# CHEBSB/PolarDecoding

Measured on AMD Instinct MI355X. Metric: decoded frames/sec, N=1024 K=512 CA-SCL L=8, higher is better.
Workload: dtype f64

## Files before the change

include/polar_hip.h:

```cpp
#ifndef POLAR_HIP_H
#define POLAR_HIP_H

#include <stddef.h>
#include <stdint.h>

#ifdef __cplusplus
extern "C" {
#endif

#define POLAR_ALGO_SC 0
#define POLAR_ALGO_BP 1
#define POLAR_ALGO_SCL 2
#define POLAR_ALGO_CASCL 3
#define POLAR_ALGO_SCF 4
#define POLAR_ALGO_SCAN 5
#define POLAR_ALGO_BPL 6

#define POLAR_F64 0
#define POLAR_F32 1
#define POLAR_Q8 2

#define POLAR_OK 0
#define POLAR_EINVAL (-1)
#define POLAR_ENOMEM (-2)
// ... 102 lines not shown

int polar_bpl_set_graphs(polar_ctx *ctx, const int *perms, int P);
int polar_bpl_get_graphs(const polar_ctx *ctx, int *P, int *perms);
int polar_bpl_cyclic_graphs(int n, int P, int *out);
int polar_bpl_decode_device(polar_ctx *ctx, const void *d_in, int in_is_f32, double sigma, size_t B, uint32_t *d_uhat_bits,
                            uint32_t *d_iters, uint32_t *d_flags, uint32_t *d_graph, uint32_t *d_total_iters);
int polar_bpl_decode_batch(polar_ctx *ctx, const double *llr_in, size_t B, int *u_hat, unsigned *iters, unsigned *flags,
                           unsigned *graph, unsigned *total_iters);

#define POLAR_RM_NONE 0
#define POLAR_RM_REPEAT 1
#define POLAR_RM_PUNCTURE 2
#define POLAR_RM_SHORTEN 3
#define POLAR_RM_SHORT_LLR 1048576.0
int polar_rm_select_n(int A, int E, int n_max);
int polar_rm_info_order(int N, int A, int E, int *out);
int polar_create_rm(const polar_cfg *cfg, int E, int ibil, polar_ctx **out);
int polar_rm_info(const polar_ctx *ctx, int *E, int *mode, int *ibil);
int polar_rm_recover_device(polar_ctx *ctx, const void *d_in, int in_is_f32, double sigma, size_t B, void *d_out);

int polar_genie_count_device(polar_ctx *ctx, const void *d_in, int in_is_f32, double sigma, size_t B, uint64_t *d_counts);
int polar_genie_rows_device(polar_ctx *ctx, unsigned long long seed, unsigned long long first_frame, double sigma, size_t B,
                            void *d_out, int out_is_f32);
int polar_construct_batch(polar_ctx *ctx, unsigned long long seed, unsigned long long first_frame, double sigma, size_t B,
                          uint64_t *d_counts);
int polar_construct_order(int N, const uint64_t *counts, const int *base_order, int *out);

typedef struct polar_dyn {
    int D;
    const int *pos;
    const int *ptr;
    const int *idx;
} polar_dyn;
int polar_create_dyn(const polar_cfg *cfg, const polar_dyn *dyn, polar_ctx **out);
int polar_dyn_info(const polar_ctx *ctx, int *D, int *pos);
int polar_dyn_pac(int N, const int *info_order, int A, const int *g_taps, int n_taps, int *pos, int *ptr, int *idx,
                  int idx_cap, int *nnz);
int polar_pac_precode(int N, const int *g_taps, int n_taps, const int *v, size_t B, int *u);
int polar_pac_unprecode(int N, const int *g_taps, int n_taps, const int *u, size_t B, int *v);
int polar_dyn_pc5g(int N, const int *q_i, int n_qi, int n_pc, int n_pc_wm, int *pos, int *ptr, int *idx, int idx_cap,
                   int *nnz, int *info_order);


int polar_transform_device(polar_ctx *ctx, const uint32_t *d_in, size_t B, uint32_t *d_out);
int polar_encode_device(polar_ctx *ctx, const uint32_t *d_payload, size_t B, uint32_t *d_u_bits, uint32_t *d_x_bits);
int polar_payload_device(polar_ctx *ctx, const uint32_t *d_uhat_bits, size_t B, uint32_t *d_payload, uint32_t *d_crc_ok);
int polar_encode_batch(polar_ctx *ctx, const int *payload, size_t B, int *u, int *x);
int polar_payload_batch(polar_ctx *ctx, const int *u_hat, size_t B, int *payload, unsigned *crc_ok);
int polar_set_systematic(polar_ctx *ctx, int on);
int polar_get_systematic(const polar_ctx *ctx);
int polar_systematic_check(int N, const int *info_order, int A);
int polar_crc_masks(int N, const int *info_order, int A, int crc_r, const int *crc_taps, int n_taps, int systematic,
                    uint32_t *crc_tab, uint32_t *masks);

int polar_q8_set_quant(polar_ctx *ctx, double scale, int qc, int qi);
int polar_q8_get_quant(const polar_ctx *ctx, double *scale, int *qc, int *qi);
int polar_q8_quantize_host(const double *in, size_t n, double sigma, double scale, int qc, int8_t *out);
int polar_q8_quantize_device(polar_ctx *ctx, const void *d_in, int in_is_f32, double sigma, size_t B, int8_t *d_out);
int polar_q8_decode_device(polar_ctx *ctx, const int8_t *d_q, size_t B, uint32_t *d_uhat_bits, int32_t *d_pm, uint32_t *d_flags);
int polar_q8_decode_batch(polar_ctx *ctx, const int8_t *q, size_t B, int *u_hat, int32_t *pm, unsigned *flags);

int polar_generate_device(polar_ctx *ctx, unsigned long long seed, unsigned long long first_frame, double snr_db,
                          size_t B, void *d_out, int out_is_f32, int out_is_y, uint32_t *d_u_bits);

int polar_fer_batch(polar_ctx *ctx, unsigned long long seed, unsigned long long first_frame, double snr_db, size_t B,
                    unsigned long long *block_errors, unsigned long long *bit_errors);

typedef struct polar_group polar_group;
int polar_group_create(const polar_cfg *cfg, int ngpus, polar_group **out);
void polar_group_destroy(polar_group *grp);
int polar_group_size(const polar_group *grp);
int polar_group_fer_batch(polar_group *grp, unsigned long long seed, unsigned long long first_frame, double snr_db,
                          size_t frames_per_gpu, unsigned long long *block_errors, unsigned long long *bit_errors,
                          double *seconds);
int polar_group_stop_rule_batch(polar_group *grp, unsigned long long seed, unsigned long long first_frame, double snr_db,
                                size_t frames_per_gpu, unsigned need, size_t min_frames, size_t *frames_used,
                                unsigned long long *block_errors, unsigned long long *bit_errors);
int polar_fer_multi_gpu(const polar_cfg *cfg, int ngpus, unsigned long long seed, unsigned long long first_frame,
                        double snr_db, size_t frames_per_gpu, unsigned long long *block_errors,
                        unsigned long long *bit_errors, double *seconds);

int polar_set_stream(polar_ctx *ctx, void *hip_stream);
void *polar_get_stream(polar_ctx *ctx);
int polar_synchronize(polar_ctx *ctx);

int polar_time_decode_device(polar_ctx *ctx, const void *d_in, int in_is_f32, double sigma, size_t B,
                             uint32_t *d_uhat_bits, int reps, float *ms_per_launch);

int polar_info_order(const polar_ctx *ctx, int *out, int n);
int polar_ctx_info(const polar_ctx *ctx, int *N, int *K, int *A, int *L, int *algo, int *dtype);
const char *polar_kernel_name(const polar_ctx *ctx);
const char *polar_version(void);

#ifdef __cplusplus
}
#endif
#endif
```

polardecoding_amd/csrc/polar_hip.hip:

```cpp
#include "polar_host.h"
#ifdef POLAR_TESTING
#include "../../include/polar_hip_testing.h"
#endif

#include <dlfcn.h>

#include <chrono>
#include <cmath>
#include <cstdio>
#include <cstdlib>
#include <mutex>
#include <thread>

#include "count_kernel.h"
#include "gen_kernel.h"
#include "scf_params.h"
#include "scan_params.h"

namespace {

const int kQ5G[1024] = {
#include "q5g_table.inc"
};

std::vector<int> default_order(int N)
{
    std::vector<int> q;
    if (N <= 1024) {
        for (int i = 0; i < 1024; ++i)
            if (kQ5G[i] < N) q.push_back(kQ5G[i]);
    } else {
        int n = 0;
        while ((1 << n) < N) ++n;
        std::vector<std::pair<double, int>> w(N);
        const double beta = std::pow(2.0, 0.25);
        for (int i = 0; i < N; ++i) {
            double s = 0;
            for (int b = 0; b < n; ++b)
                if ((i >> b) & 1) s += std::pow(beta, b);
            w[i] = {s, i};
        }
        std::stable_sort(w.begin(), w.end());
        for (auto &x : w) q.push_back(x.second);
    }
    return q;
}

std::vector<uint32_t> make_crc_table(int N, int r, const std::vector<int> &taps, const std::vector<int> &I)
{
    std::vector<uint32_t> tab(N, 0u);
    uint64_t glow = 0;
    for (int t : taps)
        if (t < r) glow |= 1ull << t;
    const uint64_t top = 1ull << r;
    uint64_t rem = 1;
    if (r == 0) return tab;
    for (size_t i = 0; i < I.size(); ++i) {
        tab[I[i]] = (uint32_t)rem;
        rem <<= 1;
        if (rem & top) rem = (rem ^ top) ^ glow;
    }
    return tab;
}

std::vector<uint32_t> make_crc_masks(int N, const std::vector<uint32_t> &tab)
{
    std::vector<uint32_t> t = tab;
    for (int s = 1; s < N; s <<= 1)
        for (int k = 0; k < N; ++k)
            if (k & s) t[(size_t)k] ^= t[(size_t)(k ^ s)];
    const int NW = N / 32;
    std::vector<uint32_t> m((size_t)polar::CRC_MASK_ROWS * NW, 0u);
    for (int k = 0; k < N; ++k)
        for (int i = 0; i < polar::CRC_MASK_ROWS; ++i)
            if ((t[(size_t)k] >> i) & 1u) m[(size_t)i * NW + (k >> 5)] |= 1u << (k & 31);
    return m;
}

int upload_crc_tables(polar_ctx *c, const std::vector<uint32_t> &t)
{
    const std::vector<uint32_t> m = make_crc_masks(c->cfg.N, t);
    if (int rc = c->d_crc_tab.upload(t.data(), t.size())) return rc;
    return c->d_crc_mask.upload(m.data(), m.size());
}

size_t chunk_rows(const polar_ctx *c, size_t B, size_t row_bytes, size_t floor = 64)
{
    return std::min(B, std::max(floor, c->chunk_bytes / row_bytes));
}

bool has_crc(int algo) { return algo == POLAR_ALGO_CASCL || algo == POLAR_ALGO_SCF || algo == POLAR_ALGO_BPL; }

const int kRmP[32] = {0, 1, 2, 4, 3, 5, 6, 7, 8, 16, 9, 17, 10, 18, 11, 19, 12, 20, 13, 21, 14, 22, 15, 23, 24, 25, 26, 28, 27, 29, 30, 31};

int rm_J(int N, int n) { return kRmP[n / (N / 32)] * (N / 32) + n % (N / 32); }

bool rm_args_ok(int N, int A, int E)
{
    return N >= 32 && N <= 1024 && !(N & (N - 1)) && A >= 1 && E >= A && E <= 8192;
}

int rm_mode_of(int N, int A, int E)
{
    if (E >= N) return POLAR_RM_REPEAT;
    return (16 * A <= 7 * E) ? POLAR_RM_PUNCTURE : POLAR_RM_SHORTEN;
}

int rm_order(int N, int A, int E, std::vector<int> &I)
{
    if (!rm_args_ok(N, A, E)) return POLAR_EINVAL;
    std::vector<unsigned char> pre((size_t)N, 0);
    const int mode = rm_mode_of(N, A, E);
    if (mode == POLAR_RM_PUNCTURE) {
        for (int n = 0; n < N - E; ++n) pre[(size_t)rm_J(N, n)] = 1;
        const int t = (4 * E >= 3 * N) ? (3 * N - 2 * E + 3) / 4 : (9 * N - 4 * E + 15) / 16;
        for (int i = 0; i < t; ++i) pre[(size_t)i] = 1;
    } else if (mode == POLAR_RM_SHORTEN) {
        for (int n = E; n < N; ++n) pre[(size_t)rm_J(N, n)] = 1;
    }
    const std::vector<int> q = default_order(N);
    I.clear();
    for (int i = N - 1; i >= 0 && (int)I.size() < A; --i)
        if (!pre[(size_t)q[(size_t)i]]) I.push_back(q[(size_t)i]);
    if ((int)I.size() < A) return POLAR_EINVAL;
    std::reverse(I.begin(), I.end());
    return POLAR_OK;
}

std::vector<uint16_t> rm_channel_ilv(int E)
// ... 103 lines not shown

int q8_decode_rows(polar_ctx *c, const void *d_in, int in_is_f32, double sigma, size_t B, uint32_t *d_bits, double *d_pm,
                   uint32_t *d_flags)
{
    const size_t esz = in_is_f32 ? 4 : 8;
    if (reinterpret_cast<uintptr_t>(d_in) % esz) return POLAR_EINVAL;
    const size_t N = (size_t)c->cfg.N;
    const size_t CH = chunk_rows(c, B, N);
    int rc;
    if ((rc = ensure(c, c->q8_rows, CH * N))) return rc;
    if (d_pm && (rc = ensure(c, c->q8_pm, CH * sizeof(int32_t)))) return rc;
    for (size_t off = 0; off < B; off += CH) {
        const size_t nc = std::min(CH, B - off);
        int8_t *rows = (int8_t *)c->q8_rows.p;
        int32_t *pm = d_pm ? (int32_t *)c->q8_pm.p : nullptr;
        if ((rc = polar_tu::q8_quantize(c, (const char *)d_in + off * N * esz, in_is_f32 != 0, sigma, nc * N, rows))) return rc;
        if ((rc = polar_tu::q8_decode(c, rows, nc, d_bits + off * (size_t)c->NW, pm, d_flags ? d_flags + off : nullptr))) return rc;
        if (d_pm && (rc = polar_tu::q8_pm_f64(c, pm, nc, d_pm + off))) return rc;
    }
    return POLAR_OK;
}

int decode_fixed(polar_ctx *c, const void *d_in, int in_is_f32, double sigma, size_t B, uint32_t *d_bits,
                 double *d_pm, uint32_t *d_flags, const uint32_t *d_frozen, uint32_t *d_iters = nullptr)
{
    if (!c || !d_in || !d_bits) return POLAR_EINVAL;
    if (B == 0) return POLAR_OK;
    if (B > 0x7fffffffull) return POLAR_EINVAL;
    const polar_cfg &g = c->cfg;
    if (g.dtype == POLAR_Q8) return q8_decode_rows(c, d_in, in_is_f32, sigma, B, d_bits, d_pm, d_flags);
    const bool f32 = g.dtype == POLAR_F32;
    const Family fam = kernel_family(c, in_is_f32, B);
    if (fam == Family::BP) {
        polar::BpParams P{};
        P.in = d_in; P.sigma = sigma; P.out_bits = d_bits; P.frozen = d_frozen;
        P.N = g.N; P.n = c->n; P.B = (int)B; P.iters = g.bp_iters;
        if (d_pm) HIP_TRY(c, hipMemsetAsync(d_pm, 0, B * sizeof(double), c->stream));
        P.stop = c->bp_stop;
        if (P.stop != POLAR_BP_STOP_NONE) {
            P.iters_out = d_iters;
            P.flags_out = d_flags;
        } else {
            if (d_flags) HIP_TRY(c, hipMemsetAsync(d_flags, 0, B * sizeof(uint32_t), c->stream));
            if (d_iters) HIP_TRY(c, hipMemsetD32Async(reinterpret_cast<hipDeviceptr_t>(d_iters), g.bp_iters, B, c->stream));
        }
        return polar_tu::bp(c, P, f32, in_is_f32 != 0);
    }
    polar::SclParams P{};
    P.in = d_in; P.sigma = sigma; P.out_bits = d_bits; P.pm = d_pm; P.flags = d_flags;
    P.frozen = d_frozen;
    P.crc_tab = (g.algo == POLAR_ALGO_CASCL) ? c->d_crc_tab : nullptr;
    P.crc_mask = (g.algo == POLAR_ALGO_CASCL) ? c->d_crc_mask : nullptr;
    P.crc_r = (g.algo == POLAR_ALGO_CASCL) ? g.crc_r : 0;
    P.N = g.N; P.n = c->n; P.B = (int)B;
    P.sc_mode = (g.algo == POLAR_ALGO_SC) ? 1 : 0;
    P.dbg = nullptr;
    P.scratch = nullptr;
    P.queue = nullptr;
    const bool in32 = in_is_f32 != 0;
    const bool crc = g.algo == POLAR_ALGO_CASCL;
    switch (fam) {
    case Family::WIDE: return polar_tu::scl_wide(c, P, f32, in32);
    case Family::DYN: return polar_tu::scl_dyn(c, P, f32, in32);
    case Family::SC_LANES: return polar_tu::sc_lanes(c, P, f32, in32);
#ifdef POLAR_TESTING
    case Family::FAST4: return polar_tu::scl_fast4(c, P, f32, in32, crc);
#endif
    case Family::FAST2: return polar_tu::scl_fast2(c, P, f32, in32, crc);
    case Family::FAST: return polar_tu::scl_fast(c, P, f32, in32, crc);
    case Family::BIG: return f32 ? polar_tu::scl_big_f32(c, P, in32) : polar_tu::scl_big_f64(c, P, in32);
    default: return polar_tu::scl_generic(c, P, f32, in32);
    }
}

void refresh_kernel_name(polar_ctx *c);
void sync_stage_ctx(polar_ctx *c)
{
    for (polar_ctx *s : c->stage_ctx) {
        if (!s) continue;
        s->stream.adopt(c->stream);
        s->force_generic = c->force_generic;
        s->force_spill = c->force_spill;
        s->use_fast2 = c->use_fast2;
        s->use_fast4 = c->use_fast4;
        s->big_split = c->big_split;
        s->chunk_bytes = c->chunk_bytes;
    }
}

int cascl_adaptive(polar_ctx *c, const void *d_in, int in_is_f32, double sigma, size_t B, uint32_t *d_bits,
                   double *d_pm, uint32_t *d_flags, uint32_t *d_list)
{
    hipStreamCaptureStatus cs = hipStreamCaptureStatusNone;
    HIP_TRY(c, hipStreamIsCapturing(c->stream, &cs));
    if (cs != hipStreamCaptureStatusNone) return POLAR_EINVAL;
    sync_stage_ctx(c);
    const std::vector<int> &st = c->cascl_stages;
    const int m = (int)st.size(), N = c->cfg.N, NW = c->NW;
    const size_t row = (size_t)N * (in_is_f32 ? 4 : 8);
    const size_t CH = chunk_rows(c, B, row);
    int rc;
    if (!d_flags) {
        if ((rc = ensure(c, c->ad_flags, B * sizeof(uint32_t)))) return rc;
        d_flags = (uint32_t *)c->ad_flags.p;
    }
    for (Buf *b : {&c->ad_idx[0], &c->ad_idx[1], &c->ad_sflags})
// ... 365 lines not shown
        }
        a += "; glue k_ad_crc_check, k_ad_fail_count/scan/write, k_ad_gather, k_ad_scatter";
        c->kernel_name = a;
    }
    if (c->rm_mode != POLAR_RM_NONE) c->kernel_name = "k_rm_recover, then " + c->kernel_name;
    if (fam == Family::DYN || (fam == Family::WIDE && c->is_dyn)) c->kernel_name = nm;
}

std::vector<uint32_t> pack_mask(const unsigned char *m, int N, bool invert)
{
    std::vector<uint32_t> w(N / 32, 0u);
    for (int j = 0; j < N; ++j)
        if ((m[j] != 0) != invert) w[j >> 5] |= 1u << (j & 31);
    return w;
}

void unpack_words(const uint32_t *w, int NW, int *out)
{
    struct Row { int v[8]; };
    static const std::vector<Row> tab = [] {
        std::vector<Row> t(256);
        for (int b = 0; b < 256; ++b)
            for (int k = 0; k < 8; ++k) t[(size_t)b].v[k] = (b >> k) & 1;
        return t;
    }();
    for (int i = 0; i < NW; ++i) {
        const uint32_t x = w[i];
        std::memcpy(out + 32 * i, &tab[x & 255u], sizeof(Row));
        std::memcpy(out + 32 * i + 8, &tab[(x >> 8) & 255u], sizeof(Row));
        std::memcpy(out + 32 * i + 16, &tab[(x >> 16) & 255u], sizeof(Row));
        std::memcpy(out + 32 * i + 24, &tab[x >> 24], sizeof(Row));
    }
}

constexpr unsigned HOST_THREADS = 6;
int host_batch(polar_ctx *c, const double *in, double sigma, const unsigned char *frozen_mask, size_t B,
               int *u_hat, double *pm_out, unsigned *flags, unsigned *iters = nullptr, unsigned *graph = nullptr,
               unsigned *total = nullptr, int *sets = nullptr)
{
    if (!c || !in || !u_hat) return POLAR_EINVAL;
    DeviceGuard guard(c->cfg.device);
    if (B == 0) return POLAR_OK;
    const int N = c->cfg.N, NW = c->NW;
    const int W = c->rm_mode != POLAR_RM_NONE ? c->rm_E : N;
    const uint32_t *d_frozen = c->d_frozen;
    if (frozen_mask) {
        if (has_crc(c->cfg.algo) || c->rm_mode != POLAR_RM_NONE || c->is_dyn || c->cfg.dtype == POLAR_Q8) return POLAR_EINVAL;
        std::vector<uint32_t> w = pack_mask(frozen_mask, N, false);
        if (!c->d_frozen_override) HIP_TRY(c, c->d_frozen_override.alloc((size_t)NW));
        HIP_TRY(c, hipMemcpyAsync(c->d_frozen_override, w.data(), NW * sizeof(uint32_t), hipMemcpyHostToDevice,
                                  c->stream));
        HIP_TRY(c, hipStreamSynchronize(c->stream));
        d_frozen = c->d_frozen_override;
    }
    int rc;
    if ((rc = ensure(c, c->pm, B * sizeof(double)))) return rc;
    if ((rc = ensure(c, c->flags, B * sizeof(uint32_t)))) return rc;
    if (iters && (rc = ensure(c, c->bp_iters, B * sizeof(uint32_t)))) return rc;
    if (graph && (rc = ensure(c, c->bpl_graph, B * sizeof(uint32_t)))) return rc;
    if (total && (rc = ensure(c, c->bpl_total, B * sizeof(uint32_t)))) return rc;
    if (sets && (rc = ensure(c, c->scf_hsets, B * polar::SCF_MAX_ORDER * sizeof(int32_t)))) return rc;
    const size_t CH = std::max<size_t>(256, std::min<size_t>(16384, ((size_t)128 << 20) / ((size_t)W * sizeof(double))));
    std::vector<size_t> off{0};
    {
        std::vector<size_t> head, tail;
        size_t left = B;
        if (B >= 6 * CH && CH >= 2048) {
            for (size_t d = 8; d >= 2; d /= 2) {
                head.push_back(CH / d);
                tail.insert(tail.begin(), CH / d);
                left -= 2 * (CH / d);
            }
        }
        for (size_t h : head) off.push_back(off.back() + h);
        while (left > 0) {
            const size_t nfc = std::min(CH, left);
            off.push_back(off.back() + nfc);
            left -= nfc;
        }
        for (size_t t : tail) off.push_back(off.back() + t);
    }
    const size_t nch = off.size() - 1;
    const size_t chf = std::min(B, CH);
    for (int i = 0; i < 2; ++i) {
        if ((rc = ensure(c, c->in2[i], chf * W * sizeof(double)))) return rc;
        if ((rc = ensure(c, c->bits2[i], chf * NW * sizeof(uint32_t)))) return rc;
    }
    const bool staged = nch >= 3;
    for (int i = 0; i < 2; ++i) {
        HIP_TRY(c, c->h_bits[i].ensure(chf * NW * sizeof(uint32_t)));
        if (staged) HIP_TRY(c, c->h_in[i].ensure(chf * W * sizeof(double)));
    }
    if (!c->copy_stream) {
        HIP_TRY(c, c->copy_stream.create(hipStreamNonBlocking));
        for (int i = 0; i < 2; ++i) {
            HIP_TRY(c, c->ev_in[i].create(hipEventDisableTiming));
            HIP_TRY(c, c->ev_free[i].create(hipEventDisableTiming));
            HIP_TRY(c, c->ev_out[i].create(hipEventDisableTiming));
        }
    }
    auto stage_chunk = [&](size_t k) {
        const size_t f0 = off[k], nf = off[k + 1] - off[k];
        const double *src = in + f0 * (size_t)W;
        double *dst = c->h_in[k & 1];
        const unsigned nthr = HOST_THREADS;
        auto part = [=](unsigned t) {
// ... 151 lines not shown
        std::vector<int> q = default_order(N);
        c->info_order.assign(q.end() - c->A, q.end());
    }
    c->cfg.info_order = c->info_order.data();
    c->frozen.assign(N, 1);
    for (int i = 0; i < c->A; ++i) {
        const int j = c->info_order[i];
        if (j < 0 || j >= N || c->frozen[j] == 0) { delete c; return POLAR_EINVAL; }
        c->frozen[j] = 0;
    }
    c->h_crc_tab = make_crc_table(N, r, c->taps, c->info_order);
    c->scf_T = std::min(8, c->A);

    int ndev = 0;
    if (hipGetDeviceCount(&ndev) != hipSuccess || cfg->device < 0 || cfg->device >= ndev) {
        delete c;
        return POLAR_EDEVICE;
    }
    DeviceGuard guard(cfg->device);
    hipDeviceProp_t prop;
    hipError_t e = hipGetDeviceProperties(&prop, cfg->device);
    if (e != hipSuccess) {
        delete c;
        return POLAR_EDEVICE;
    }
    c->num_cu = prop.multiProcessorCount;
    auto cleanup = [&](int rc) {
        polar_destroy(c);
        return rc;
    };
    if (c->stream.create(hipStreamNonBlocking) != hipSuccess) return cleanup(POLAR_EDEVICE);
    if (c->ev0.create(hipEventDefault) != hipSuccess || c->ev1.create(hipEventDefault) != hipSuccess) return cleanup(POLAR_EDEVICE);
    std::vector<uint32_t> fw = pack_mask(c->frozen.data(), N, false);
    std::vector<uint32_t> iw = pack_mask(c->frozen.data(), N, true);
    c->cfg.crc_systematic = (cfg->crc_systematic && r > 0) ? 1 : 0;
    if (c->cfg.crc_systematic) {
        std::fill(iw.begin(), iw.end(), 0u);
        for (int i = r; i < c->A; ++i) iw[c->info_order[i] >> 5] |= 1u << (c->info_order[i] & 31);
        std::vector<uint32_t> rows((size_t)cfg->K);
        uint64_t glow = 0;
        for (int t : c->taps)
            if (t < r) glow |= 1ull << t;
        const uint64_t top = 1ull << r;
        uint64_t rem = glow;
        for (int k = 0; k < cfg->K; ++k) {
            rows[(size_t)k] = (uint32_t)rem;
            rem <<= 1;
            if (rem & top) rem = (rem ^ top) ^ glow;
        }
        if (int rc = c->d_gc_rows.upload(rows.data(), rows.size())) return cleanup(rc);
    }
    if (c->d_frozen.alloc((size_t)c->NW) != hipSuccess || c->d_info.alloc((size_t)c->NW) != hipSuccess) return cleanup(POLAR_ENOMEM);
    if (int rc = c->d_frozen.upload(fw.data(), (size_t)c->NW)) return cleanup(rc);
    if (int rc = c->d_info.upload(iw.data(), (size_t)c->NW)) return cleanup(rc);
    if (r > 0)
        if (int rc = upload_crc_tables(c, c->h_crc_tab)) return cleanup(rc);
    if (cfg->algo == POLAR_ALGO_BPL) {
        c->bp_stop = POLAR_BP_STOP_G;
        const int P = std::min(c->n, 8);
        std::vector<int> perms((size_t)P * c->n);
        polar_bpl_cyclic_graphs(c->n, P, perms.data());
        if (int rc = polar_bpl_set_graphs(c, perms.data(), P)) return cleanup(rc);
    }
    refresh_kernel_name(c);
    *out = c;
    return POLAR_OK;
}

void polar_destroy(polar_ctx *c)
{
    if (!c) return;
    DeviceGuard guard(c->cfg.device);
    for (hipStream_t st : {c->stream.get(), c->copy_stream.get(), c->lane_b.stream.get()})
        if (st) (void)hipStreamSynchronize(st);
    for (polar_ctx *s : c->stage_ctx) polar_destroy(s);
    delete c;
}

int polar_set_stream(polar_ctx *c, void *s)
{
    if (!c) return POLAR_EINVAL;
    DeviceGuard guard(c->cfg.device);
    if (c->stream.is_owned()) (void)hipStreamSynchronize(c->stream);
    c->stream.adopt((hipStream_t)s);
    return POLAR_OK;
}

void *polar_get_stream(polar_ctx *c) { return c ? (void *)c->stream.get() : nullptr; }

int polar_synchronize(polar_ctx *c)
{
    if (!c) return POLAR_EINVAL;
    DeviceGuard guard(c->cfg.device);
    HIP_TRY(c, hipStreamSynchronize(c->stream));
    return POLAR_OK;
}

int polar_ctx_info(const polar_ctx *c, int *N, int *K, int *A, int *L, int *algo, int *dtype)
{
    if (!c) return POLAR_EINVAL;
    if (N) *N = c->cfg.N;
    if (K) *K = c->cfg.K;
    if (A) *A = c->A;
    if (L) *L = c->cfg.L;
    if (algo) *algo = c->cfg.algo;
    if (dtype) *dtype = c->cfg.dtype;
// ... 962 lines not shown
            if (j & s) t[(size_t)j] ^= t[(size_t)(j ^ s)];
    for (int j = 0; j < N; ++j)
        if (c->frozen[(size_t)j]) t[(size_t)j] = 0u;
}

}

int polar_systematic_check(int N, const int *info_order, int A)
{
    if (N < 32 || N > 4096 || (N & (N - 1)) || !info_order || A < 1 || A > N) return POLAR_EINVAL;
    const int NW = N / 32;
    std::vector<uint32_t> keep((size_t)NW, 0u);
    for (int i = 0; i < A; ++i) {
        const int j = info_order[i];
        if (j < 0 || j >= N || ((keep[(size_t)(j >> 5)] >> (j & 31)) & 1u)) return POLAR_EINVAL;
        keep[(size_t)(j >> 5)] |= 1u << (j & 31);
    }
    std::vector<uint32_t> w((size_t)NW);
    for (int i = 0; i < A; ++i) {
        const int j = info_order[i];
        std::fill(w.begin(), w.end(), 0u);
        w[(size_t)(j >> 5)] = 1u << (j & 31);
        host_transform(w.data(), NW);
        for (int k = 0; k < NW; ++k) w[(size_t)k] &= keep[(size_t)k];
        host_transform(w.data(), NW);
        for (int k = 0; k < NW; ++k)
            if ((w[(size_t)k] & keep[(size_t)k]) != (k == (j >> 5) ? 1u << (j & 31) : 0u)) return 0;
    }
    return 1;
}

int polar_crc_masks(int N, const int *info_order, int A, int crc_r, const int *crc_taps, int n_taps, int systematic,
                    uint32_t *crc_tab, uint32_t *masks)
{
    if (N < 32 || N > 4096 || (N & (N - 1)) || !info_order || A < 1 || A > N || crc_r < 1 || crc_r > 32 || !crc_taps ||
        n_taps < 2 || !masks)
        return POLAR_EINVAL;
    polar_ctx c;
    c.cfg.N = N;
    c.frozen.assign((size_t)N, 1);
    for (int i = 0; i < A; ++i) {
        if (info_order[i] < 0 || info_order[i] >= N) return POLAR_EINVAL;
        c.frozen[(size_t)info_order[i]] = 0;
    }
    c.h_crc_tab = make_crc_table(N, crc_r, std::vector<int>(crc_taps, crc_taps + n_taps), std::vector<int>(info_order, info_order + A));
    std::vector<uint32_t> t = c.h_crc_tab;
    if (systematic) make_crc_table_sys(&c, t);
    if (crc_tab) std::copy(t.begin(), t.end(), crc_tab);
    const std::vector<uint32_t> m = make_crc_masks(N, t);
    std::copy(m.begin(), m.end(), masks);
    return POLAR_OK;
}

int polar_get_systematic(const polar_ctx *c) { return c && c->sys_polar ? 1 : 0; }

int polar_set_systematic(polar_ctx *c, int on)
{
    if (!c || (on != 0 && on != 1)) return POLAR_EINVAL;
    if ((on != 0) == c->sys_polar) return POLAR_OK;
    if (on) {
        if (c->is_dyn || c->rm_mode != POLAR_RM_NONE || c->cfg.dtype == POLAR_Q8 || c->cfg.algo == POLAR_ALGO_BPL) return POLAR_EINVAL;
        if (polar_systematic_check(c->cfg.N, c->info_order.data(), c->A) != 1) return POLAR_EINVAL;
    }
    DeviceGuard guard(c->cfg.device);
    if (c->d_crc_tab) {
        if (c->h_crc_tab_sys.empty()) make_crc_table_sys(c, c->h_crc_tab_sys);
        const std::vector<uint32_t> &t = on ? c->h_crc_tab_sys : c->h_crc_tab;
        HIP_TRY(c, hipStreamSynchronize(c->stream));
        if (int rc = upload_crc_tables(c, t)) return rc;
        for (polar_ctx *s : c->stage_ctx)
            if (s && s->d_crc_tab)
                if (int rc = upload_crc_tables(s, t)) return rc;
    }
    c->sys_polar = on != 0;
    return POLAR_OK;
}

int polar_transform_device(polar_ctx *c, const uint32_t *d_in, size_t B, uint32_t *d_out)
{
    if (!c || !d_in || !d_out || B > 0x7fffffffull) return POLAR_EINVAL;
    DeviceGuard guard(c->cfg.device);
    return polar_tu::enc_transform(c, d_in, nullptr, false, B, d_out);
}

int polar_encode_device(polar_ctx *c, const uint32_t *d_payload, size_t B, uint32_t *d_u_bits, uint32_t *d_x_bits)
{
    if (!c || !d_payload || (!d_u_bits && !d_x_bits) || B > 0x7fffffffull) return POLAR_EINVAL;
    if (B == 0) return POLAR_OK;
    DeviceGuard guard(c->cfg.device);
    int rc;
    if ((rc = enc_tables(c))) return rc;
    const size_t row = (size_t)c->NW * sizeof(uint32_t);
    uint32_t *u = d_u_bits;
    if (!u) {
        if ((rc = ensure_nomem(c, c->enc_u, B * row, kEncScratch))) return rc;
        u = (uint32_t *)c->enc_u.p;
    }
    const bool rm = c->rm_mode != POLAR_RM_NONE;
    if (rm && d_x_bits && (rc = ensure_nomem(c, c->enc_x, B * row, kEncScratch))) return rc;
    if ((rc = polar_tu::enc_place(c, d_payload, B, u))) return rc;
    if (c->is_dyn && (rc = polar_tu::enc_dyn_fill(c, u, B))) return rc;
    if (c->sys_polar && (rc = polar_tu::enc_transform(c, u, nullptr, true, B, u))) return rc;
    if (!d_x_bits) return POLAR_OK;
    if (!rm) return polar_tu::enc_transform(c, u, nullptr, false, B, d_x_bits);
    if ((rc = polar_tu::enc_transform(c, u, nullptr, false, B, (uint32_t *)c->enc_x.p))) return rc;
    return polar_tu::enc_rm_select(c, (const uint32_t *)c->enc_x.p, B, d_x_bits);
// ... 432 lines not shown
```

polardecoding_amd/csrc/polar_host.h:

```cpp
#pragma once
#include "../../include/polar_hip.h"

#include <hip/hip_runtime.h>

#include <algorithm>
#include <cstdint>
#include <cstring>
#include <string>
#include <vector>

#include "dev_owned.h"
#include "polar_params.h"

namespace polar {
struct ScfParams;
struct GenParams;
struct ScanParams;
}

struct Lane {
    Stream stream;
    Buf scratch;
    Buf rm_rows;
    Buf q8_rows;
};

constexpr size_t kChunkBytes = (size_t)256 << 20;

struct polar_ctx : Lane {
    polar_cfg cfg{};
    int n = 0, A = 0, NW = 0, logL = 0;
    std::vector<int> info_order;
    std::vector<unsigned char> frozen;
    std::vector<int> taps;
    std::vector<uint32_t> h_crc_tab;
    Stream copy_stream;
    Lane lane_b;
    Event ev_b;
    Event ev_in[2], ev_free[2], ev_out[2];
    Event ev0, ev1;
    DevMem<uint32_t> d_frozen;
    DevMem<uint32_t> d_info;
    DevMem<uint32_t> d_crc_tab;
    DevMem<uint32_t> d_crc_mask;
    DevMem<uint32_t> d_gc_rows;
    DevMem<uint32_t> d_frozen_override;
    DevMem<int> d_info_order;
    int num_cu = 0;
    Buf in, bits, pm, flags;
    Buf bp_iters;
    int bp_stop = POLAR_BP_STOP_NONE;
    std::vector<int> cascl_stages;
    std::vector<polar_ctx *> stage_ctx;
    Buf ad_flags;
    Buf ad_idx[2], ad_blk, ad_cnt;
    Buf ad_in, ad_bits, ad_pm, ad_sflags;
    int scf_T = 8;
    Buf scf_flips, scf_pass, scf_bits;
    int scf_omega = 0, scf_Tk[3] = {0, 0, 0};
    double scf_c = 0.0, scf_tau = 0.0;
    Buf scf_sets[2], scf_lkey, scf_lpos, scf_lcnt, scf_spass, scf_surv;
    Buf scf_hsets;
    std::vector<int> bpl_perms;
    std::vector<unsigned char> bpl_ident;
    DevMem<uint16_t> d_bpl_sigma, d_bpl_sinv;
    DevMem<uint32_t> d_bpl_frozen;
    DevMem<uint32_t> d_bpl_crc;
    Buf bpl_siters, bpl_graph, bpl_total;
    int scan_I = 4;
    Buf scan_llr, scan_ext;
    int rm_E = 0, rm_mode = POLAR_RM_NONE, rm_ibil = 0;
    DevMem<uint16_t> d_rm_ilv, d_rm_ilv_inv;
    Buf genie_rows;
    bool is_dyn = false;
    std::vector<int> dyn_pos;
    DevMem<uint32_t> d_dyn_mask;
    DevMem<int> d_dyn_row, d_dyn_pos;
    bool sys_polar = false;
    DevMem<uint16_t> d_enc_inv;
    DevMem<uint32_t> d_enc_rtab;
    std::vector<uint32_t> h_crc_tab_sys;
    Buf enc_u, enc_x, enc_io;
    double q8_scale = 2.0;
    int q8_qc = 8, q8_qi = 8;
    Buf q8_pm;
    Buf in2[2], bits2[2];
    PinnedMem<uint32_t> h_bits[2];
    PinnedMem<double> h_in[2];
    Buf gen_llr, gen_u, gen_cnt;
    std::string last_error;
    std::string kernel_name;
    bool force_generic = false;
    bool use_fast2 = true;
    bool use_fast4 = false;
    bool force_spill = false;
    int big_split = 0;
    size_t chunk_bytes = kChunkBytes;
};

// ... 172 lines not shown
```

polardecoding_amd/csrc/polar_params.h:

```cpp
#pragma once
#include <stdint.h>

namespace polar {

constexpr int CRC_MASK_ROWS = 32;

struct SclParams {
    const void *in;
    double sigma;
    uint32_t *out_bits;
    double *pm;
    uint32_t *flags;
    const uint32_t *frozen;
    const uint32_t *crc_tab;
    int N, n;
    int B;
    int sc_mode;
    void *scratch;
    unsigned long long *dbg;
    unsigned *queue;
    const uint32_t *crc_mask;
    int crc_r;
};

struct BpParams {
    const void *in;
    double sigma;
    uint32_t *out_bits;
    const uint32_t *frozen;
    int N, n, B, iters;
    unsigned *queue;
    int stop;
    uint32_t *iters_out;
    uint32_t *flags_out;
};
constexpr uint32_t BP_FLAG_CONVERGED = 0x8u;

struct BpReadoutParams {
    const void *in;
    double sigma;
    uint32_t *out_bits;
    const uint32_t *frozen;
    const uint32_t *info;
    const uint32_t *u_bits;
    unsigned long long *E;
    int cp[8];
    int ncp;
    int N, n, B, iters;
};

#ifdef __HIPCC__
__device__ __forceinline__ unsigned job_fetch(unsigned *queue, int total)
{
    const unsigned nx = atomicAdd(queue, 1u);
    if (nx == (unsigned)(total - 1)) atomicExch(queue, 0u);
    return nx;
}
__device__ __forceinline__ int next_job_wave(unsigned *queue, int cur, int resident, int total)
{
    if (!queue) return cur + resident;
    unsigned nx = 0;
    if ((threadIdx.x & 63) == 0) nx = job_fetch(queue, total);
    return resident + (int)__builtin_amdgcn_readfirstlane(nx);
}
__device__ __forceinline__ int next_job_block(unsigned *queue, int cur, int resident, int total, int *slot)
{
    if (!queue) return cur + resident;
    if (threadIdx.x == 0) *slot = (int)job_fetch(queue, total);
    __syncthreads();
    const int nx = *slot;
    __syncthreads();
    return resident + nx;
}
#endif

// ... 3 lines not shown
```

polardecoding_amd/csrc/scl_fast2.h:

```cpp
#pragma once
#include "scl_fast.h"

namespace polar {

template <typename R>
struct Fast2Cfg {
    static constexpr int NLOG = 10, N = 1024, NW = 32, TOP = 9, HI = 8, L = 8;
    static constexpr int NA = 32;
    static constexpr int WAVES = 4;
    static constexpr int MIN_WAVES_PER_SIMD = sizeof(R) == 8 ? 3 : 4;
    static constexpr int NFA = HI - 3;
    static constexpr size_t sc_l8 = 0;
    static constexpr size_t sc_l7 = sc_l8 + 8 * 256;
    static constexpr size_t sc_l6 = sc_l7 + 8 * 128;
    static constexpr size_t sc_tl = sc_l6 + 8 * 64;
    static constexpr size_t scratch_cw = sc_tl + 512;
    static constexpr size_t scratch_elems = 2 * scratch_cw;
    static constexpr size_t off_lut = 0;
    static constexpr size_t off_frz = off_lut + ((Lut<R>::bytes + 15) / 16) * 16;
    static constexpr size_t off_msk = off_frz + 4 * NW;
    static constexpr size_t off_kth = off_msk + 4 * CRC_MASK_ROWS * NW;
    static constexpr size_t off_stair = off_kth + 256 * 8;
    static constexpr size_t shared_bytes = off_stair + ((Stair<R>::bytes + 15) / 16) * 16;
    static constexpr size_t off_bl = 0;
// ... 393 lines not shown
    template <int K, bool FULL>
    __device__ __forceinline__ void decide_t(int o, bool frozen, R lam, R tt)
    {
        if (frozen) {
            PM += tt + negmax(lam);
            set_bit_k<K>(o, 0u);
            return;
        }
        uint32_t bit;
        R pm;
        if (!FULL && logact < 3) {
            const R ph0 = tt + negmax(lam), ph1 = tt + posmax(lam);
            bit = (p >> logact) & 1;
            pm = PM + (bit ? ph1 : ph0);
            ++logact;
        } else {
            const uint32_t lneg = sign_bit(lam);
            const R cb = PM + tt, cw = PM + (tt + absr(lam));
            bit = (uint32_t)dpp_i<0x00>((int)lneg);
            pm = cb;
            if (!trivial_prune(cb, cw)) ranked<K>(lneg, cb, cw, bit, pm);
        }
        PM = pm;
        set_bit_k<K>(o, bit);
    }
    template <int K>
    __device__ __forceinline__ void ranked(uint32_t lneg, R cb, R cw, uint32_t &bit, R &pm)
    {
        const R c0 = lneg ? cw : cb, c1 = lneg ? cb : cw;
        const uint32_t mask = survivors(c0, c1);
        const uint32_t m0 = mask & 0xFFu, m1 = mask >> 8;
        const uint32_t m_both = m0 & m1, m_dead = ~(m0 | m1) & 0xFFu;
        if (__popc(mask) < L) fl |= 0x1u;
        const bool s0 = (m0 >> p) & 1, s1 = (m1 >> p) & 1;
        bit = (!s0 && s1) ? 1u : 0u;
        pm = bit ? c1 : c0;
        if (__ballot(m_dead != 0u) == 0ull) return;
        const bool dead = !s0 && !s1;
        const int myrank = __popc(m_dead & ((1u << p) - 1u));
        const bool refilled = dead && (myrank < __popc(m_both));
        const int src = (int)kth[m_both * 8 + myrank];
        const int sg = refilled ? src : p;
        const int sl = sg * 8 + gl;
        const R c1s = __shfl(c1, sl);
        ptr = __shfl(ptr, sl);
        bl0 = __shfl(bl0, sl);
        if constexpr ((K & 4) == 0) { A[2] = __shfl(A[2], sl); A[3] = __shfl(A[3], sl); }
        if constexpr ((K & 2) == 0) { A[1] = __shfl(A[1], sl); a1 = __shfl(a1, sl); }
        if constexpr ((K & 1) == 0) { bp_d = __shfl(bp_d, sl); bp_td = __shfl(bp_td, sl); }
        bit = refilled ? 1u : bit;
        pm = refilled ? c1s : pm;
    }

    __device__ __forceinline__ void frozen_prefix(int P)
    {
        const int w32 = p * 4 + pos, j0 = 8 * P;
        vm_drain();
        {
            const SPtr tl = tls();
            const SPtr o8 = l8(0), o7 = l7(0);
            R v8[8];
#pragma unroll
            for (int k = 0; k < 8; ++k) {
                const int e = w32 + 32 * k;
                v8[k] = chk(ld_sc(tl + e), ld_sc(tl + e + 256));
                o8[e] = v8[k];
            }
            lds_fence();
#pragma unroll
            for (int k = 0; k < 4; ++k) {
                const R v7 = chk(v8[k], v8[k + 4]);
                o7[w32 + 32 * k] = v7;
                stg[w32 + 32 * k] = v7;
            }
            set_pa(8, 0);
            set_pa(7, 0);
        }
        lds_fence();
#pragma unroll
        for (int t = 6; t >= 0; --t) {
            const int h = 1 << t;
            int idx[2];
            R x[2], y[2];
#pragma unroll
            for (int i = 0; i < 2; ++i) {
                const int b = w32 + 32 * i;
                idx[i] = ((b >> t) << (t + 1)) | (b & (h - 1));
                x[i] = stg[idx[i]];
                y[i] = stg[idx[i] + h];
            }
            lds_fence();
#pragma unroll
            for (int i = 0; i < 2; ++i) {
                stg[idx[i]] = chk(x[i], y[i]);
                stg[idx[i] + h] = y[i] + x[i];
            }
            lds_fence();
            if (t >= 4) {
                const R *node = stg + ((j0 >> t) << t) + pos;
#pragma unroll
                for (int r = 0; r < h / 4; ++r) A[h / 4 + r] = node[4 * r];
            }
        }
#pragma unroll
        for (int k = 0; k < 4; ++k) {
            const R lam = stg[w32 + 32 * k];
            stg[128 + w32 + 32 * k] = lut.tabv(lam) + negmax(lam);
        }
        lds_fence();
        R pm = PM;
#pragma unroll 8
        for (int j = 0; j < j0; ++j) pm += stg[128 + j];
        PM = pm;
        lds_fence();
    }

    template <bool FULL>
    __device__ __forceinline__ void octet_frozen_prefix(int o, bool last_frozen)
    {
        R xf = chks(A[2], A[3]), xg = A[3] + A[2];
        R yf = quadp<0x4E>(xf), yg = quadp<0x4E>(xg);
        {
            const R ff = chks(xf, yf), gf = xf + yf, fg = chks(xg, yg), gg = xg + yg;
            xf = (pos & 2) ? gf : ff;
            xg = (pos & 2) ? gg : fg;
        }
        yf = quadp<0xB1>(xf); yg = quadp<0xB1>(xg);
        R lf, lg;
        {
            const R ff = chks(xf, yf), gf = xf + yf, fg = chks(xg, yg), gg = xg + yg;
            lf = (pos & 1) ? gf : ff;
            lg = (pos & 1) ? gg : fg;
        }
        const R pf = lut.tabv(lf) + negmax(lf), pg = lut.tabv(lg) + negmax(lg);
        PM += pf;
        PM += quadp<0x55>(pf);
        PM += quadp<0xAA>(pf);
        PM += quadp<0xFF>(pf);
        PM += pg;
        PM += quadp<0x55>(pg);
        PM += quadp<0xAA>(pg);
        bl0 &= ~0xFEu;
        if (last_frozen) {
            PM += quadp<0xFF>(pg);
            set_bit7(o, 0u);
        } else {
            decide<7, FULL>(o, false, quadp<0xFF>(lg));
        }
    }

    struct ChkBp { R v, s, d, ts, td; };
    __device__ __forceinline__ ChkBp chk_bp(R x, R y) const
    {
        ChkBp r;
        r.s = x + y;
        r.d = x - y;
        r.ts = lut.tabv(r.s);
        r.td = lut.tabv(r.d);
        r.v = xor_sign(minabs(x, y), x, y) + (r.ts - r.td);
        return r;
    }
    static __device__ __forceinline__ R g_sel(R sum, R dif, uint32_t w, int sh)
    {
        const uint32_t m = (uint32_t)__builtin_amdgcn_sbfe((int)w, sh, 1);
        return Lut<R>::sel_mask(m, -dif, sum);
    }
    template <int K, bool FULL>
// ... 62 lines not shown
    unsigned char *base = smem + C::shared_bytes + (size_t)wave * C::per_wave;
    uint32_t *frz = reinterpret_cast<uint32_t *>(smem + C::off_frz);
    uint32_t *msk = reinterpret_cast<uint32_t *>(smem + C::off_msk);
    unsigned char *kth = smem + C::off_kth;

    Lut<R>::build(smem + C::off_lut, threadIdx.x, blockDim.x);
    for (int i = threadIdx.x; i < NW; i += blockDim.x) frz[i] = P.frozen[i];
    if (CRC_ON)
        for (int i = threadIdx.x; i < CRC_MASK_ROWS * NW; i += blockDim.x)
            msk[i] = P.crc_mask[(i & ~(NW - 1)) + ((i >> 3) & 3) + 4 * (i & 7)];
    for (int i = threadIdx.x; i < 256 * 8; i += blockDim.x) {
        int m = i >> 3, k = i & 7, idx = 0, seen = 0;
        for (int b = 0; b < 8; ++b)
            if ((m >> b) & 1) {
                if (seen == k) idx = b;
                ++seen;
            }
        kth[i] = (unsigned char)idx;
    }
    __syncthreads();

    D s;
    s.lane = threadIdx.x & 63;
    s.p = s.lane >> 3;
    s.c = (s.lane >> 2) & 1;
    s.pos = s.lane & 3;
    s.pos0_mask = s.pos == 0 ? 0xFFFFFFFFu : 0u;
    s.gl = s.lane & 7;
    s.lut.bind(smem + C::off_lut);
    s.kth = kth;
    s.blw = reinterpret_cast<uint32_t *>(base + C::off_bl) + s.c * 8 * NW;
    s.curw = reinterpret_cast<uint32_t *>(base + C::off_cw) + s.c * 8 * NW;
    s.cand = reinterpret_cast<R *>(base + C::off_cd) + s.c * 16;
    s.keys = reinterpret_cast<uint32_t *>(base + C::off_ky) + s.c * 16;
    s.stg = reinterpret_cast<R *>(base + C::off_sg) + s.c * 256;
    if constexpr (FROM_Y) s.sigma = P.sigma;
    {
        const int i = s.lane & 15, row = s.lane >> 4, cwr = row >> 1, h = row & 1;
        const int jj = (i + 8 * h) & 15;
        s.own_addr = 64 * cwr + 4 * (2 * (i & 7) + (i >> 3));
        s.oth_addr = 64 * cwr + 4 * (2 * (jj & 7) + (jj >> 3));
        s.cand_addr = (int)sizeof(R) * 16 * cwr;
    }
    const int lane = s.lane, p = s.p, c = s.c, pos = s.pos;
    const int wave_global = blockIdx.x * C::WAVES + wave;
    const int waves_total = gridDim.x * C::WAVES;
    R *scr_wave = reinterpret_cast<R *>(P.scratch) + (size_t)wave_global * C::scratch_elems;
    s.rs_scr = D::make_rsrc(scr_wave, (unsigned)(C::scratch_elems * sizeof(R)));
    s.cscr = (unsigned)c * (unsigned)C::scratch_cw;

    int lead = 0;
    while (lead < 15 && ((frz[lead >> 2] >> (8 * (lead & 3))) & 0xFFu) == 0xFFu) ++lead;
    lead = __builtin_amdgcn_readfirstlane(lead);

    for (int pair = wave_global; 2 * pair < P.B;) {
        const int frame_raw = 2 * pair + c;
        const bool live = frame_raw < P.B;
        const int frame = live ? frame_raw : P.B - 1;
        s.rs_in = D::make_rsrc(reinterpret_cast<const IN *>(P.in) + (size_t)(2 * pair) * N, (unsigned)(2 * N * sizeof(IN)));
        s.csrc = (unsigned)(frame - 2 * pair) * (unsigned)N;
        {
            const auto t = s.tls();
            const int w = p * 4 + pos;
#pragma unroll 2
            for (int e = w; e < N / 2; e += 32) t[e] = s.chk(s.chv(e), s.chv(e + N / 2));
        }
        for (int w = lane; w < 2 * 8 * NW; w += 64) (s.blw - c * 8 * NW)[w] = 0;
        lds_fence();

        s.PM = R(0);
        s.ptr = 0;
        for (int t = 4; t <= 8; ++t) s.set_pa(t, p);
        for (int t = 5; t <= 9; ++t) s.set_pb(t, p);
        s.bl0 = 0;
        s.a1 = R(0);
#pragma unroll
        for (int r = 0; r < C::NA; ++r) s.A[r] = R(0);
        s.fl = 0;
        s.logact = 0;
        uint32_t fword = 0;

        int o_first = 0;
        if (lead > 0) {
            s.frozen_prefix(lead);
            o_first = lead;
            fword = frz[o_first >> 2];
        }
        int o = o_first;
#pragma unroll 1
        while (o < N / 8 && s.logact < 3) o = octet_group<D, false>(s, frz, fword, o);
        while (o < N / 8) o = octet_group<D, true>(s, frz, fword, o);

        bool pass = false;
        if constexpr (CRC_ON) {
            lds_fence();
            uint32_t x[8];
#pragma unroll
            for (int j = 0; j < 8; ++j) x[j] = s.curw[p * NW + pos + 4 * j];
            typedef uint32_t u4_t __attribute__((ext_vector_type(4)));
            const u4_t *mk = reinterpret_cast<const u4_t *>(msk + 8 * pos);
            const int rows = (P.crc_r + 3) & ~3;
            uint32_t rem = 0;
#pragma unroll 1
            for (int i = 0; i < rows; i += 4) {
#pragma unroll
                for (int k = 0; k < 4; ++k) {
                    const u4_t a = mk[(i + k) * (NW / 4)], b = mk[(i + k) * (NW / 4) + 1];
                    const uint32_t acc = (x[0] & a.x) ^ (x[1] & a.y) ^ (x[2] & a.z) ^ (x[3] & a.w) ^ (x[4] & b.x) ^
                                         (x[5] & b.y) ^ (x[6] & b.z) ^ (x[7] & b.w);
                    rem |= (uint32_t)(__popc(acc) & 1) << (i + k);
                }
            }
            rem ^= (uint32_t)dpp_i<0xB1>((int)rem);
            rem ^= (uint32_t)dpp_i<0x4E>((int)rem);
            pass = rem == 0u;
        }
        const uint64_t bp_ = __ballot(pass && pos == 0);
        const uint64_t cwmask = 0x0101010101010101ull << (4 * c);
        const bool any = (bp_ & cwmask) != 0ull;
        int best = -1;
        R best_pm = R(0);
        for (int q = 0; q < L; ++q) {
            const R pq = __shfl(s.PM, q * 8 + 4 * c);
            const int okq = __shfl((int)(any ? pass : true), q * 8 + 4 * c);
            if (okq && (best < 0 || pq < best_pm)) {
                best = q;
                best_pm = pq;
            }
        }
        uint32_t fl = s.fl;
        if (any) fl |= 0x2u;
        lds_fence();
        {
            const int w = p * 4 + pos;
            uint32_t x = s.curw[best * NW + w];
            x ^= (x >> 1) & 0x55555555u;
            x ^= (x >> 2) & 0x33333333u;
            x ^= (x >> 4) & 0x0F0F0F0Fu;
// ... 32 lines not shown
```

Baseline: 14.29 million.

## Add specialized fill phase for sparse-info leading region in fast2 SCL

Adds a host-side analysis that detects when the first 128–256 bits of an N=1024 code contain at most three info bits, all at the ends of 64-bit blocks. In that case the kernel decodes the region with a dedicated routine. The routine computes whole 64-leaf subtrees in LDS, sums the frozen-bit penalties in bulk and handles only the last two leaves per block bit by bit. The goal is to replace many octet-group iterations and their list bookkeeping with a streamlined pass while the list is still small. It adds new code paths and host state for override masks, and it only applies to frozen patterns that match the detector.

```diff
diff --git a/include/polar_hip.h b/include/polar_hip.h
--- a/include/polar_hip.h
+++ b/include/polar_hip.h
@@ -178,6 +178,7 @@
 int polar_systematic_check(int N, const int *info_order, int A);
 int polar_crc_masks(int N, const int *info_order, int A, int crc_r, const int *crc_taps, int n_taps, int systematic,
                     uint32_t *crc_tab, uint32_t *masks);
+int polar_fill_phase_end(int N, const int *info_order, int A);
 
 int polar_q8_set_quant(polar_ctx *ctx, double scale, int qc, int qi);
 int polar_q8_get_quant(const polar_ctx *ctx, double *scale, int *qc, int *qi);
diff --git a/polardecoding_amd/csrc/polar_hip.hip b/polardecoding_amd/csrc/polar_hip.hip
--- a/polardecoding_amd/csrc/polar_hip.hip
+++ b/polardecoding_amd/csrc/polar_hip.hip
@@ -75,6 +75,32 @@
         for (int i = 0; i < polar::CRC_MASK_ROWS; ++i)
             if ((t[(size_t)k] >> i) & 1u) m[(size_t)i * NW + (k >> 5)] |= 1u << (k & 31);
     return m;
+}
+
+int fill_phase_end(int N, const unsigned char *frozen)
+{
+    if (N != 1024) return 0;
+    int lead = 0;
+    while (lead < 15) {
+        bool all = true;
+        for (int k = 0; k < 8; ++k) all = all && frozen[8 * lead + k] != 0;
+        if (!all) break;
+        ++lead;
+    }
+    for (int E = 256; E >= 128; E -= 64) {
+        int count = 0, early = 0, first = 0;
+        bool ok = true;
+        for (int j = 0; j < E; ++j) {
+            if (frozen[j]) continue;
+            if ((j & 63) < 62 || j < 126) ok = false;
+            ++count;
+            if (j < E - 64) ++early;
+            if (j < 128) ++first;
+        }
+        if (E > 128 && !(first == 1 && early == 1)) ok = false;
+        if (ok && count <= 3 && E > 8 * lead) return E;
+    }
+    return 0;
 }
 
 int upload_crc_tables(polar_ctx *c, const std::vector<uint32_t> &t)
@@ -284,6 +310,7 @@
     P.crc_tab = (g.algo == POLAR_ALGO_CASCL) ? c->d_crc_tab : nullptr;
     P.crc_mask = (g.algo == POLAR_ALGO_CASCL) ? c->d_crc_mask : nullptr;
     P.crc_r = (g.algo == POLAR_ALGO_CASCL) ? g.crc_r : 0;
+    P.fill_end = d_frozen == c->d_frozen ? c->fill_end : d_frozen == c->d_frozen_override ? c->fill_end_override : 0;
     P.N = g.N; P.n = c->n; P.B = (int)B;
     P.sc_mode = (g.algo == POLAR_ALGO_SC) ? 1 : 0;
     P.dbg = nullptr;
@@ -755,6 +782,7 @@
                                   c->stream));
         HIP_TRY(c, hipStreamSynchronize(c->stream));
         d_frozen = c->d_frozen_override;
+        c->fill_end_override = fill_phase_end(N, frozen_mask);
     }
     int rc;
     if ((rc = ensure(c, c->pm, B * sizeof(double)))) return rc;
@@ -1012,6 +1040,7 @@
     }
     if (c->d_frozen.alloc((size_t)c->NW) != hipSuccess || c->d_info.alloc((size_t)c->NW) != hipSuccess) return cleanup(POLAR_ENOMEM);
     if (int rc = c->d_frozen.upload(fw.data(), (size_t)c->NW)) return cleanup(rc);
+    c->fill_end = fill_phase_end(N, c->frozen.data());
     if (int rc = c->d_info.upload(iw.data(), (size_t)c->NW)) return cleanup(rc);
     if (r > 0)
         if (int rc = upload_crc_tables(c, c->h_crc_tab)) return cleanup(rc);
@@ -2080,6 +2109,17 @@
     return POLAR_OK;
 }
 
+int polar_fill_phase_end(int N, const int *info_order, int A)
+{
+    if (N < 32 || N > 4096 || (N & (N - 1)) || !info_order || A < 1 || A > N) return POLAR_EINVAL;
+    std::vector<unsigned char> frozen((size_t)N, 1);
+    for (int i = 0; i < A; ++i) {
+        if (info_order[i] < 0 || info_order[i] >= N) return POLAR_EINVAL;
+        frozen[(size_t)info_order[i]] = 0;
+    }
+    return fill_phase_end(N, frozen.data());
+}
+
 int polar_get_systematic(const polar_ctx *c) { return c && c->sys_polar ? 1 : 0; }
 
 int polar_set_systematic(polar_ctx *c, int on)
diff --git a/polardecoding_amd/csrc/polar_host.h b/polardecoding_amd/csrc/polar_host.h
--- a/polardecoding_amd/csrc/polar_host.h
+++ b/polardecoding_amd/csrc/polar_host.h
@@ -45,6 +45,7 @@
     DevMem<uint32_t> d_crc_mask;
     DevMem<uint32_t> d_gc_rows;
     DevMem<uint32_t> d_frozen_override;
+    int fill_end = 0, fill_end_override = 0;
     DevMem<int> d_info_order;
     int num_cu = 0;
     Buf in, bits, pm, flags;
diff --git a/polardecoding_amd/csrc/polar_params.h b/polardecoding_amd/csrc/polar_params.h
--- a/polardecoding_amd/csrc/polar_params.h
+++ b/polardecoding_amd/csrc/polar_params.h
@@ -21,6 +21,7 @@
     unsigned *queue;
     const uint32_t *crc_mask;
     int crc_r;
+    int fill_end;
 };
 
 struct BpParams {
diff --git a/polardecoding_amd/csrc/scl_fast2.h b/polardecoding_amd/csrc/scl_fast2.h
--- a/polardecoding_amd/csrc/scl_fast2.h
+++ b/polardecoding_amd/csrc/scl_fast2.h
@@ -469,7 +469,7 @@
         pm = refilled ? c1s : pm;
     }
 
-    __device__ __forceinline__ void frozen_prefix(int P)
+    __device__ __forceinline__ void frozen_prefix(int P, int nphi, bool regs, R &xl, R &yl)
     {
         const int w32 = p * 4 + pos, j0 = 8 * P;
         vm_drain();
@@ -506,6 +506,10 @@
                 x[i] = stg[idx[i]];
                 y[i] = stg[idx[i] + h];
             }
+            if (t == 0) {
+                xl = stg[126];
+                yl = stg[127];
+            }
             lds_fence();
 #pragma unroll
             for (int i = 0; i < 2; ++i) {
@@ -513,7 +517,7 @@
                 stg[idx[i] + h] = y[i] + x[i];
             }
             lds_fence();
-            if (t >= 4) {
+            if (t >= 4 && regs) {
                 const R *node = stg + ((j0 >> t) << t) + pos;
 #pragma unroll
                 for (int r = 0; r < h / 4; ++r) A[h / 4 + r] = node[4 * r];
@@ -527,9 +531,117 @@
         lds_fence();
         R pm = PM;
 #pragma unroll 8
-        for (int j = 0; j < j0; ++j) pm += stg[128 + j];
+        for (int j = 0; j < nphi; ++j) pm += stg[128 + j];
         PM = pm;
         lds_fence();
+    }
+
+    __device__ __forceinline__ uint32_t fill_tail(uint32_t f2, R lam0, R xl, R yl)
+    {
+        uint32_t b0 = 0, b1 = 0;
+        if (!(f2 & 1u)) {
+            b0 = (p >> logact) & 1;
+            ++logact;
+        }
+        PM += lut.tabv(lam0) + (b0 ? posmax(lam0) : negmax(lam0));
+        const R lam1 = b0 ? -(xl - yl) : yl + xl;
+        if (!(f2 & 2u)) {
+            b1 = (p >> logact) & 1;
+            ++logact;
+        }
+        PM += lut.tabv(lam1) + (b1 ? posmax(lam1) : negmax(lam1));
+        return (b0 ? 0x55555555u : 0u) ^ (b1 ? 0xFFFFFFFFu : 0u);
+    }
+    __device__ __forceinline__ void fill_phase(int E, const uint32_t *frz, R xl, R yl)
+    {
+        const int w32 = (int)fresh((unsigned)(p * 4 + pos));
+        const int qb = (p & 1) * 64;
+        const uint32_t wv0 = fill_tail(frz[3] >> 30, stg[126], xl, yl);
+        uint32_t wv1 = 0;
+        lds_fence();
+        blw[p * NW + 4 + pos] = wv0;
+        lds_fence();
+#pragma unroll 1
+        for (int S = 128; S < E; S += 64) {
+            vm_drain();
+            const uint32_t wsel = S == 128 ? wv0 : wv1;
+            uint32_t wq[2];
+            wq[0] = (uint32_t)__shfl((int)wsel, gl) >> w32;
+            wq[1] = (uint32_t)__shfl((int)wsel, 8 + gl) >> w32;
+            if (S == 128) {
+                const SPtr s8 = l8(0) + w32;
+                R v8[8];
+#pragma unroll
+                for (int k = 0; k < 8; ++k) v8[k] = ld_sc(s8 + 32 * k);
+#pragma unroll
+                for (int q = 0; q < 2; ++q) {
+                    const SPtr o7 = l7(q) + w32;
+                    R v7[4];
+#pragma unroll
+                    for (int k = 0; k < 4; ++k) {
+                        v7[k] = g_bit<R>(v8[k], v8[k + 4], wq[q], 0);
+                        o7[32 * k] = v7[k];
+                    }
+                    stg[64 * q + w32] = chk(v7[0], v7[2]);
+                    stg[64 * q + w32 + 32] = chk(v7[1], v7[3]);
+                }
+                set_pa(7, p & 1);
+            } else {
+#pragma unroll
+                for (int q = 0; q < 2; ++q) {
+                    const SPtr s7 = l7(q) + w32;
+#pragma unroll
+                    for (int i = 0; i < 2; ++i)
+                        stg[64 * q + w32 + 32 * i] = g_bit<R>(ld_sc(s7 + 32 * i), ld_sc(s7 + 32 * i + 64), wq[q], 0);
+                }
+            }
+            lds_fence();
+#pragma unroll
+            for (int t = 5; t >= 0; --t) {
+                const int h = 1 << t;
+                int idx[2];
+                R x[2], y[2];
+#pragma unroll
+                for (int i = 0; i < 2; ++i) {
+                    const int b = w32 + 32 * i;
+                    idx[i] = ((b >> t) << (t + 1)) | (b & (h - 1));
+                    x[i] = stg[idx[i]];
+                    y[i] = stg[idx[i] + h];
+                }
+                if (t == 0) {
+                    xl = stg[qb + 62];
+                    yl = stg[qb + 63];
+                }
+                lds_fence();
+#pragma unroll
+                for (int i = 0; i < 2; ++i) {
+                    stg[idx[i]] = chk(x[i], y[i]);
+                    stg[idx[i] + h] = y[i] + x[i];
+                }
+                lds_fence();
+            }
+#pragma unroll
+            for (int k = 0; k < 4; ++k) {
+                const R lam = stg[w32 + 32 * k];
+                stg[128 + w32 + 32 * k] = lut.tabv(lam) + negmax(lam);
+            }
+            lds_fence();
+            R pm = PM;
+#pragma unroll 2
+            for (int j = 0; j < 62; ++j) pm += stg[128 + qb + j];
+            PM = pm;
+            const uint32_t wv = fill_tail(frz[(S + 62) >> 5] >> 30, stg[qb + 62], xl, yl);
+            lds_fence();
+            if (S == 128) {
+                wv1 = wv;
+                if (pos < 2) blw[p * NW + 2 + pos] = wv;
+            } else {
+                const uint32_t b = pos < 2 ? wv1 ^ wv : wv;
+                blw[p * NW + 8 + pos] = wv0 ^ b;
+                blw[p * NW + 12 + pos] = b;
+            }
+            lds_fence();
+        }
     }
 
     template <bool FULL>
@@ -698,6 +810,7 @@
     int lead = 0;
     while (lead < 15 && ((frz[lead >> 2] >> (8 * (lead & 3))) & 0xFFu) == 0xFFu) ++lead;
     lead = __builtin_amdgcn_readfirstlane(lead);
+    const int E = P.fill_end;
 
     for (int pair = wave_global; 2 * pair < P.B;) {
         const int frame_raw = 2 * pair + c;
@@ -727,9 +840,14 @@
         uint32_t fword = 0;
 
         int o_first = 0;
-        if (lead > 0) {
-            s.frozen_prefix(lead);
+        if (E > 0 || lead > 0) {
+            R xl, yl;
+            s.frozen_prefix(E > 0 ? 15 : lead, E > 0 ? 126 : 8 * lead, E == 0, xl, yl);
             o_first = lead;
+            if (E > 0) {
+                s.fill_phase(E, frz, xl, yl);
+                o_first = E >> 3;
+            }
             fword = frz[o_first >> 2];
         }
         int o = o_first;
```

New measurement: 14.83 million (median of 6 runs). 3.8% higher.
